# rail-berkeley/serl

Measured on AMD Instinct MI355X. Metric: learner grad-steps/sec (DrQ, bs256, 2x128x128 img), higher is better.
Workload: dtype f32 (trunk convs as split-fp16 MFMA x3, fp32 accumulate; <=1e-6 vs fp64); 1 GPU; async_drq_sim (DrQ, ResNet-10 frozen trunk, REDQ-10 critic); workload_key=drq, global_batch=256, per_gpu_batch=256, cameras=2, state_dim=24, act_dim=6, replay_capacity=200000, replay_fill=20000, parallelism=dp1, encoder=resnet-pretrained, trunk_passes_per_grad_step=2, trunk_arithmetic=f16x3, schedule=trunk(i+1) overlapped with update(i) on a 2nd stream; gather(i+2) on a 3rd

## Files before the change

serl_amd/csrc/heads.hip:

```cpp
#include <algorithm>
#include <cstdlib>

#include "heads.h"
#include "jaxrng.h"
#include "ln_stats.h"
#include "prof.h"

namespace serl {

long g_chain_launches = 0;
#define SERL_LAUNCH_CHAIN(...) do { ++g_chain_launches; hipLaunchKernelGGL(__VA_ARGS__); } while (0)

typedef float f32x16 __attribute__((ext_vector_type(16)));

constexpr int kGBM = 64, kGBN = 64, kGBK = 32, kGP = 36, kGPT = 68;
constexpr int kGTile = kGBM * kGP;
static_assert(kGBK * kGPT <= kGTile, "the [k][row] layout must fit the tile");
typedef float f32x4 __attribute__((ext_vector_type(4)));
typedef float f32x4u __attribute__((ext_vector_type(4), aligned(4)));

__device__ __forceinline__ f32x4 ld4(const float* p, int valid) {
  f32x4 v = {0.f, 0.f, 0.f, 0.f};
  if (valid >= 4) {
    v = *reinterpret_cast<const f32x4u*>(p);
// ... 1072 lines not shown
  for (int i = 0; i < n; ++i) {
    mv.v[i] = vs[i];
    gx = std::max(gx, cdiv(vs[i].D, 64));
    gy = std::max(gy, vs[i].groups);
  }
  SERL_LAUNCH_CHAIN(colsum3_kernel, dim3(gx, gy, n), dim3(512), 0, stream, mv);
  SERL_HIP(hipGetLastError());
  return SERL_OK;
}

int colsum3(const float* dg, const float* xhat, const float* dpre, int groups, int rows_per_group, int D,
            float* o_gamma, float* o_beta, float* o_bias, long gstride, hipStream_t stream) {
  const Colsum3Args v{dg, xhat, dpre, groups, rows_per_group, D, o_gamma, o_beta, o_bias, gstride, 0};
  return colsum3_multi(&v, 1, stream);
}

__global__ __launch_bounds__(256) void sle_fwd_kernel(Multi<SleFwdArgs> mv, float keep_scale, int N, int HW, int Cc,
                                                     long xs, long ks, long ms, long fs) {
  const long e = (long)blockIdx.x * 256 + threadIdx.x;
  if (e >= (long)N * Cc) return;
  const SleFwdArgs& v = mv.v[blockIdx.z];
  const float* x = v.x + blockIdx.y * xs;
  const float* K = v.K + blockIdx.y * ks;
  float* f = v.f + blockIdx.y * fs;
  const uint8_t* mask = v.mask ? v.mask + blockIdx.y * ms : nullptr;
  const int n = (int)(e / Cc), c = (int)(e - (long)n * Cc);
  float acc[8] = {0, 0, 0, 0, 0, 0, 0, 0};
#pragma unroll 4
  for (int hw = 0; hw < HW; ++hw) {
    const float xv = x[((long)n * HW + hw) * Cc + c];
    const float4 k0 = *reinterpret_cast<const float4*>(K + ((long)hw * Cc + c) * 8);
    const float4 k1 = *reinterpret_cast<const float4*>(K + ((long)hw * Cc + c) * 8 + 4);
    acc[0] += xv * k0.x; acc[1] += xv * k0.y; acc[2] += xv * k0.z; acc[3] += xv * k0.w;
    acc[4] += xv * k1.x; acc[5] += xv * k1.y; acc[6] += xv * k1.z; acc[7] += xv * k1.w;
  }
  float* o = f + (long)n * Cc * 8 + (long)c * 8;
  if (mask) {
    const uint8_t* m = mask + (long)n * Cc * 8 + (long)c * 8;
#pragma unroll
    for (int j = 0; j < 8; ++j) acc[j] = m[j] ? acc[j] * keep_scale : 0.f;
  }
  *reinterpret_cast<float4*>(o) = make_float4(acc[0], acc[1], acc[2], acc[3]);
  *reinterpret_cast<float4*>(o + 4) = make_float4(acc[4], acc[5], acc[6], acc[7]);
}

int sle_fwd_multi(const SleFwdArgs* vs, int n, float keep_scale, int N, int HW, int Cc, int groups, long x_gs, long k_gs,
                  long mask_gs, long f_gs, hipStream_t stream) {
  SERL_REQUIRE(n >= 1 && n <= kMaxMulti, "bad instance count %d", n);
  Multi<SleFwdArgs> mv{};
  for (int i = 0; i < n; ++i) mv.v[i] = vs[i];
  SERL_LAUNCH_CHAIN(sle_fwd_kernel, dim3(cdiv((long)N * Cc, 256), groups, n), dim3(256), 0, stream, mv, keep_scale, N,
                     HW, Cc, x_gs, k_gs, mask_gs, f_gs);
  SERL_HIP(hipGetLastError());
  return SERL_OK;
}


__device__ __forceinline__ void proprio_row(const ProprioArgs& a, int S, int row, int lane) {
  float v = a.b[lane];
  for (int s0 = 0; s0 < S; s0 += 64) {
    const float mine = (s0 + lane < S) ? a.state[(long)row * S + s0 + lane] : 0.f;
    const int cnt = min(64, S - s0);
    int s = 0;
    for (; s + 8 <= cnt; s += 8) {
      float w[8];
#pragma unroll
      for (int j = 0; j < 8; ++j) w[j] = a.W[(s0 + s + j) * 64 + lane];
#pragma unroll
      for (int j = 0; j < 8; ++j) v += __shfl(mine, s + j) * w[j];
    }
    for (; s < cnt; ++s) v += __shfl(mine, s) * a.W[(s0 + s) * 64 + lane];
  }
  float s1 = v, s2 = v * v;
  wave_sum2(s1, s2);
  float mean, rstd;
  ln_mean_rstd<64>(s1, s2, mean, rstd);
  const float xh = (v - mean) * rstd;
  a.y[(long)row * a.ld_y + lane] = tanhf(xh * a.gamma[lane] + a.beta[lane]);
  if (a.xhat) a.xhat[(long)row * 64 + lane] = xh;
  if (a.rstd && lane == 0) a.rstd[row] = rstd;
  if (a.copy_dst && lane < a.copy_cols) a.copy_dst[(long)row * a.ld_copy_dst + lane] = a.copy_src[(long)row * a.ld_copy_src + lane];
}

template <int kSleNb>
__global__ __launch_bounds__(256) void sle_proprio_fwd_kernel(Multi<SleFwdArgs> mv, Multi<ProprioArgs> pv, int has_proprio,
                                                              float keep_scale, unsigned keep_thr, float keep_p, int N, int HW, int Cc,
                                                              long xs, long ks, long ms, long fs, int S, int nb_sle) {
  if ((int)blockIdx.x >= nb_sle) {
    if (!has_proprio || blockIdx.y != 0) return;
    const int row = ((int)blockIdx.x - nb_sle) * 4 + (threadIdx.x >> 6);
    if (row < N) proprio_row(pv.v[blockIdx.z], S, row, threadIdx.x & 63);
    return;
  }
  const SleFwdArgs& v = mv.v[blockIdx.z];
  const int cblocks = (Cc + 255) / 256;
  const int c = ((int)blockIdx.x % cblocks) * 256 + threadIdx.x, n0 = ((int)blockIdx.x / cblocks) * kSleNb;
  if (c >= Cc) return;
  const float* x = v.x + blockIdx.y * xs + (long)n0 * HW * Cc + c;
  const float* K = v.K + blockIdx.y * ks + (long)c * 8;
  const int ns = min(kSleNb, N - n0);
  float acc[kSleNb][8];
#pragma unroll
  for (int s = 0; s < kSleNb; ++s)
#pragma unroll
    for (int j = 0; j < 8; ++j) acc[s][j] = 0.f;
  for (int hw0 = 0; hw0 < HW; hw0 += 4) {
    float4 k0[4], k1[4];
#pragma unroll
    for (int i = 0; i < 4; ++i) {
      const int hw = min(hw0 + i, HW - 1);
      k0[i] = *reinterpret_cast<const float4*>(K + (long)hw * Cc * 8);
      k1[i] = *reinterpret_cast<const float4*>(K + (long)hw * Cc * 8 + 4);
    }
    float xv[kSleNb][4];
#pragma unroll
    for (int s = 0; s < kSleNb; ++s)
#pragma unroll
      for (int i = 0; i < 4; ++i) xv[s][i] = x[((long)min(s, ns - 1) * HW + min(hw0 + i, HW - 1)) * Cc];
#pragma unroll
    for (int i = 0; i < 4; ++i) {
      if (hw0 + i < HW) {
#pragma unroll
        for (int s = 0; s < kSleNb; ++s) {
          acc[s][0] += xv[s][i] * k0[i].x; acc[s][1] += xv[s][i] * k0[i].y; acc[s][2] += xv[s][i] * k0[i].z; acc[s][3] += xv[s][i] * k0[i].w;
          acc[s][4] += xv[s][i] * k1[i].x; acc[s][5] += xv[s][i] * k1[i].y; acc[s][6] += xv[s][i] * k1[i].z; acc[s][7] += xv[s][i] * k1[i].w;
        }
      }
    }
  }
  float* f = v.f + blockIdx.y * fs + (long)n0 * Cc * 8 + (long)c * 8;
  const uint8_t* mask = v.mask ? v.mask + blockIdx.y * ms + (long)n0 * Cc * 8 + (long)c * 8 : nullptr;
#pragma unroll
  for (int s = 0; s < kSleNb; ++s) {
    if (s >= ns) break;
    if (mask) {
      const uint8_t* m = mask + (long)s * Cc * 8;
#pragma unroll
      for (int j = 0; j < 8; ++j) acc[s][j] = m[j] ? acc[s][j] * keep_scale : 0.f;
    } else if (v.gen == 2) {
      const uint32_t k0 = v.tf_key[blockIdx.y][0], k1 = v.tf_key[blockIdx.y][1];
      const uint64_t rowlen = (uint64_t)Cc * 8ull, total = (uint64_t)v.tf_rows * rowlen;
      const uint64_t e0 = (uint64_t)(v.tf_row0 + n0 + s) * rowlen + (uint64_t)c * 8ull;
#pragma unroll
      for (int j = 0; j < 8; ++j)
        acc[s][j] = bits_to_unit(random_bits_at(k0, k1, total, e0 + (uint64_t)j)) < keep_p ? acc[s][j] * keep_scale : 0.f;
    } else if (v.gen) {
      const uint64_t ctr = (((uint64_t)blockIdx.y * (uint64_t)v.rows_global + (uint64_t)(v.row_offset + n0 + s)) * (uint64_t)Cc + (uint64_t)c) * 3ull;
      const uint64_t h0 = mix64(v.seed ^ mix64(ctr)), h1 = mix64(v.seed ^ mix64(ctr + 1)), h2 = mix64(v.seed ^ mix64(ctr + 2));
      const unsigned u[8] = {(unsigned)(h0 & 0xFFFFFF), (unsigned)((h0 >> 24) & 0xFFFFFF), (unsigned)((h0 >> 48) | ((h1 & 0xFF) << 16)),
                             (unsigned)((h1 >> 8) & 0xFFFFFF), (unsigned)((h1 >> 32) & 0xFFFFFF), (unsigned)((h1 >> 56) | ((h2 & 0xFFFF) << 8)),
                             (unsigned)((h2 >> 16) & 0xFFFFFF), (unsigned)(h2 >> 40)};
#pragma unroll
      for (int j = 0; j < 8; ++j) acc[s][j] = u[j] < keep_thr ? acc[s][j] * keep_scale : 0.f;
    }
    *reinterpret_cast<float4*>(f + (long)s * Cc * 8) = make_float4(acc[s][0], acc[s][1], acc[s][2], acc[s][3]);
    *reinterpret_cast<float4*>(f + (long)s * Cc * 8 + 4) = make_float4(acc[s][4], acc[s][5], acc[s][6], acc[s][7]);
  }
}

int sle_proprio_fwd_multi(const SleFwdArgs* vs, const ProprioArgs* ps, int n, float keep, int N, int HW, int Cc, int groups, long x_gs,
                          long k_gs, long mask_gs, long f_gs, int state_dim, hipStream_t stream) {
  SERL_REQUIRE(n >= 1 && n <= kMaxMulti, "bad instance count %d", n);
  Multi<SleFwdArgs> mv{};
  Multi<ProprioArgs> pv{};
  for (int i = 0; i < n; ++i) {
    mv.v[i] = vs[i];
    if (ps) { pv.v[i] = ps[i]; SERL_REQUIRE(!ps[i].copy_dst || ps[i].copy_cols <= 64, "copy_cols > 64"); }
  }
  const int nb = N <= 64 ? 2 : 8;
  const int nb_sle = cdiv(Cc, 256) * cdiv(N, nb), nb_prop = ps ? cdiv(N, 4) : 0;
  if (nb == 2)
    SERL_LAUNCH_CHAIN(sle_proprio_fwd_kernel<2>, dim3(nb_sle + nb_prop, groups, n), dim3(256), 0, stream, mv, pv, ps ? 1 : 0,
                      1.0f / keep, (unsigned)(keep * 16777216.0f), keep, N, HW, Cc, x_gs, k_gs, mask_gs, f_gs, state_dim, nb_sle);
  else
    SERL_LAUNCH_CHAIN(sle_proprio_fwd_kernel<8>, dim3(nb_sle + nb_prop, groups, n), dim3(256), 0, stream, mv, pv, ps ? 1 : 0,
                      1.0f / keep, (unsigned)(keep * 16777216.0f), keep, N, HW, Cc, x_gs, k_gs, mask_gs, f_gs, state_dim, nb_sle);
  SERL_HIP(hipGetLastError());
  return SERL_OK;
}

__global__ __launch_bounds__(256) void sle_bwd_kernel(const float* x, const float* df, float* partial, int N,
                                                     int HW, int Cc, int nsplit, long x_gs, long df_gs, long part_gs) {
  const int c = blockIdx.x * 256 + threadIdx.x, hw = blockIdx.y, sp = blockIdx.z % nsplit, grp = blockIdx.z / nsplit;
  if (c >= Cc) return;
  x += grp * x_gs; df += grp * df_gs; partial += grp * part_gs;
  const int per = (N + nsplit - 1) / nsplit;
  const int nb = sp * per, ne = min(N, nb + per);
  float acc[8] = {0, 0, 0, 0, 0, 0, 0, 0};
  for (int n = nb; n < ne; ++n) {
    const float xv = x[((long)n * HW + hw) * Cc + c];
    const float4 d0 = *reinterpret_cast<const float4*>(df + (long)n * Cc * 8 + (long)c * 8);
    const float4 d1 = *reinterpret_cast<const float4*>(df + (long)n * Cc * 8 + (long)c * 8 + 4);
    acc[0] += xv * d0.x; acc[1] += xv * d0.y; acc[2] += xv * d0.z; acc[3] += xv * d0.w;
    acc[4] += xv * d1.x; acc[5] += xv * d1.y; acc[6] += xv * d1.z; acc[7] += xv * d1.w;
  }
  float* o = partial + (((long)sp * HW + hw) * Cc + c) * 8;
  *reinterpret_cast<float4*>(o) = make_float4(acc[0], acc[1], acc[2], acc[3]);
  *reinterpret_cast<float4*>(o + 4) = make_float4(acc[4], acc[5], acc[6], acc[7]);
}

__global__ __launch_bounds__(256) void sle_bwd_fused_kernel(const float* x, const float* df, float* partial, int N, int HW, int Cc,
                                                           int nsplit, long x_gs, long df_gs, long part_gs, float* out, long out_gs,
                                                           int* ctr) {
  __shared__ int s_last;
  const int c = blockIdx.x * 256 + threadIdx.x, hw = blockIdx.y, sp = blockIdx.z % nsplit, grp = blockIdx.z / nsplit;
  x += grp * x_gs; df += grp * df_gs; partial += grp * part_gs;
  const int per = (N + nsplit - 1) / nsplit;
  const int nb = sp * per, ne = min(N, nb + per);
  float acc[8] = {0, 0, 0, 0, 0, 0, 0, 0};
  if (c < Cc) {
    for (int n = nb; n < ne; ++n) {
      const float xv = x[((long)n * HW + hw) * Cc + c];
      const float4 d0 = *reinterpret_cast<const float4*>(df + (long)n * Cc * 8 + (long)c * 8);
      const float4 d1 = *reinterpret_cast<const float4*>(df + (long)n * Cc * 8 + (long)c * 8 + 4);
      acc[0] += xv * d0.x; acc[1] += xv * d0.y; acc[2] += xv * d0.z; acc[3] += xv * d0.w;
      acc[4] += xv * d1.x; acc[5] += xv * d1.y; acc[6] += xv * d1.z; acc[7] += xv * d1.w;
    }
    const __amdgpu_buffer_rsrc_t rs = rsrc_of(partial);
    const long o = (((long)sp * HW + hw) * Cc + c) * 8;
    __builtin_amdgcn_raw_buffer_store_b128(__builtin_bit_cast(u32x4_t, (f32x4){acc[0], acc[1], acc[2], acc[3]}), rs, (int)(o * 4), 0, kSc1);
    __builtin_amdgcn_raw_buffer_store_b128(__builtin_bit_cast(u32x4_t, (f32x4){acc[4], acc[5], acc[6], acc[7]}), rs, (int)(o * 4 + 16), 0, kSc1);
  }
  if (!arrive_is_last(ctr + ((long)grp * HW + hw) * gridDim.x + blockIdx.x, nsplit, &s_last)) return;
  if (c >= Cc) return;
  const __amdgpu_buffer_rsrc_t rs = rsrc_of(partial);
  f32x4 s0 = {0.f, 0.f, 0.f, 0.f}, s1 = {0.f, 0.f, 0.f, 0.f};
  for (int s = 0; s < nsplit; ++s) {
    const long o = (((long)s * HW + hw) * Cc + c) * 8;
    s0 += ld_sc1(rs, o);
    s1 += ld_sc1(rs, o + 4);
  }
  float* o = out + grp * out_gs + ((long)hw * Cc + c) * 8;
  *reinterpret_cast<f32x4*>(o) = s0;
  *reinterpret_cast<f32x4*>(o + 4) = s1;
}

int sle_bwd_fused(const float* x, const float* df, float* partial, int N, int HW, int Cc, int nsplit, int groups,
                  long x_gs, long df_gs, long part_gs, float* out, long out_gs, int* ctr, hipStream_t stream) {
  SERL_REQUIRE((long)nsplit * HW * Cc * 8 * 4 < (1L << 31), "SLE partial sums exceed 2 GB");
  SERL_LAUNCH_CHAIN(sle_bwd_fused_kernel, dim3(cdiv(Cc, 256), HW, nsplit * groups), dim3(256), 0, stream, x, df, partial, N,
                     HW, Cc, nsplit, x_gs, df_gs, part_gs, out, out_gs, ctr);
  SERL_HIP(hipGetLastError());
  return SERL_OK;
}

int sle_bwd(const float* x, const float* df, float* partial, int N, int HW, int Cc, int nsplit, int groups,
            long x_gs, long df_gs, long part_gs, hipStream_t stream) {
  SERL_LAUNCH_CHAIN(sle_bwd_kernel, dim3(cdiv(Cc, 256), HW, nsplit * groups), dim3(256), 0, stream, x, df, partial, N,
                     HW, Cc, nsplit, x_gs, df_gs, part_gs);
  SERL_HIP(hipGetLastError());
  return SERL_OK;
}

__global__ __launch_bounds__(256) void critic_loss_kernel(LossArgs L) {
  __shared__ float red[4][256];
  critic_loss_body(L, red);
}

// ... 374 lines not shown
```

serl_amd/csrc/trunk_f16x3.hip:

```cpp
#include "trunk_f16x3_elementwise.h"

namespace serl {

static int resident_workgroups(hipStream_t stream) {
  thread_local hipStream_t last = nullptr;
  thread_local int last_n = -1;
  if (last_n >= 0 && last == stream) return last_n;
  int dev = 0, n = 0;
  hipDeviceProp_t prop;
  if (hipGetDevice(&dev) == hipSuccess && hipGetDeviceProperties(&prop, dev) == hipSuccess) n = prop.multiProcessorCount;
  uint32_t mask[16] = {0};
  if (hipExtStreamGetCUMask(stream, 16, mask) == hipSuccess) {
    int m = 0;
    for (uint32_t w : mask) m += __builtin_popcount(w);
    if (m > 0 && (n == 0 || m < n)) n = m;
  } else {
    (void)hipGetLastError();
  }
  last = stream; last_n = n;
  return n;
}

static_assert(kStageFilters[0] % 64 == 0 && kStageFilters[1] % 64 == 0 && kStageFilters[2] % 64 == 0 && kStageFilters[3] % 64 == 0,
              "conv channels unsupported (Cin % 32, Cout % 64)");
// ... 31 lines not shown
    const int tiles_n = a.Cout / 64;
    if (fuse && a.P == 256) {
      l.fused = 2;
    } else if (fuse && a.P % 256 == 0 && fused_can_wait(resident, a.P / 256 * tiles_n)) {
      l.fused = 1; l.expected = a.P / 256; l.group = a.P / 256 * tiles_n;
    }
    l.stagger = (l.fused && a.M / 256 * tiles_n >= 1024) ? 5 : 0;
  } else if (dma_ok) {
    l.kern = 'D'; l.cfg = cfg;
    const int tn = cfg == 0 ? 2 : 1, tiles_n = a.Cout / (64 * tn);
    if (pmode == 1 && cfg == 4) pmode = 3;
    if (fuse && pmode == 0 && a.P % 128 == 0 && a.Cout / kGnGroups <= 64 * tn && fused_can_wait(resident, a.P / 128 * tiles_n)) {
      l.fused = 1; l.expected = a.P / 128; l.group = a.P / 128 * tiles_n;
    } else if (fuse && pmode == 0 && a.P == 64 && a.M % 128 == 0 && tn == 2 && a.Cout / kGnGroups == 64) {
      l.fused = 2;
    } else if (fuse && pmode == 2 && a.P == 16 && a.M % 128 == 0 && tn == 2 && a.Cout / kGnGroups == 128) {
      l.fused = 2;
    }
    l.proj = proj && pmode != 3 && a.KH == 3 && a.stride == 2 && a.pad == 0 && a.padw == 0;
  } else {
    l.kern = 'R'; l.cfg = cfg;
  }
  l.pmode = pmode;
  l.pad = a.pad; l.padw = a.padw;
  return l;
}

static int plan_pass(TrunkPlan& p, const TrunkDims& d, int N, const TrunkPacked& pk, const bool (&has_proj)[kTrunkStages], int resident,
                     bool fuse, bool proj_fuse) {
  p = TrunkPlan{};
  p.images = N; p.fuse = fuse;
  const bool fuse_pool = d.h[0] % 16 == 0 && d.w[0] % 16 == 0;
  const bool complete_pool = fuse_pool && N >= 512 && N % 512 == 0;
  p.pool = complete_pool ? 2 : (fuse_pool ? 1 : 0);
  const ConvArgs b0 = conv_geom(d, N, 0, 0);
  p.raw_b0 = complete_pool && fuse && !has_proj[0] && rowslab_shape_ok(b0) && b0.Cin <= 128 && pk.blk[0][0].dma && pk.blk[0][1].dma &&
             b0.P % 256 == 0 && fused_can_wait(resident, b0.P / 256 * (b0.Cout / 64));
  for (int i = 0; i < kTrunkStages; ++i) {
    TrunkPlan::L* l = p.conv[i];
    const bool raw = i == 0 && p.raw_b0;
    l[0] = plan_conv(conv_geom(d, N, i, 0), pk.blk[i][0].dma, pk.zero, fuse, resident, raw, has_proj[i] && proj_fuse && pk.blk[i][2].dma);
    if (l[0].proj) {
      l[2] = l[0];
      l[2].kern = 'F'; l[2].fused = 0;
    } else if (has_proj[i]) {
      l[2] = plan_conv(conv_geom(d, N, i, 2), pk.blk[i][2].dma, pk.zero, false, resident, false, false);
    }
    l[1] = plan_conv(conv_geom(d, N, i, 1), pk.blk[i][1].dma, pk.zero, fuse, resident, false, false);
    SERL_REQUIRE(!raw || (l[0].kern == 'S' && l[0].fused && l[1].fused),
                 "block 0 was planned on the fused row-slab path");
  }
  return SERL_OK;
}

template <int WM, int WN, int TM, int TN, int DEEP>
static void launch_igemm(ConvArgsB ab, int pmode, hipStream_t stream) {
  constexpr int BM = 32 * TM * WM, BN = 32 * TN * WN;
  ab.c.tiles_m = cdiv(ab.c.M, BM); ab.c.tiles_n = ab.c.Cout / BN;
  const dim3 grid(ab.c.tiles_m * ab.c.tiles_n), block(256);
  const size_t lds = (size_t)2 * (2 * BM * 64 + 2 * BN * 64);
  if (pmode == 0) hipLaunchKernelGGL((conv_igemm_f16x3_kernel<WM, WN, TM, TN, 0, DEEP>), grid, block, lds, stream, ab);
  else if (pmode == 1) hipLaunchKernelGGL((conv_igemm_f16x3_kernel<WM, WN, TM, TN, 1, DEEP>), grid, block, lds, stream, ab);
  else if (pmode == 2) hipLaunchKernelGGL((conv_igemm_f16x3_kernel<WM, WN, TM, TN, 2, DEEP>), grid, block, lds, stream, ab);
  else hipLaunchKernelGGL((conv_igemm_f16x3_kernel<WM, WN, TM, TN, 3, DEEP>), grid, block, lds, stream, ab);
}
template <int TN, bool PROJ>
static void launch_dma(ConvArgsB ab, int pmode, const uint8_t* zero_page, const ConvProjB& pj, hipStream_t stream) {
  ab.c.tiles_m = cdiv(ab.c.M, 128); ab.c.tiles_n = ab.c.Cout / (64 * TN);
  const dim3 grid(ab.c.tiles_m * ab.c.tiles_n), block(256);
  const size_t lds = (size_t)4 * (128 * 64 + 64 * TN * 64);
  if (pmode == 0) hipLaunchKernelGGL((conv_dma_f16x3_kernel<TN, 0, PROJ>), grid, block, lds, stream, ab, zero_page, pj);
  else if (pmode == 1) hipLaunchKernelGGL((conv_dma_f16x3_kernel<TN, 1, PROJ>), grid, block, lds, stream, ab, zero_page, pj);
  else if (pmode == 2 || PROJ) hipLaunchKernelGGL((conv_dma_f16x3_kernel<TN, 2, PROJ>), grid, block, lds, stream, ab, zero_page, pj);
  else if constexpr (!PROJ) hipLaunchKernelGGL((conv_dma_f16x3_kernel<TN, 3, false>), grid, block, lds, stream, ab, zero_page, pj);
}
static int launch_conv_f16x3(const char* tag, const TrunkPlan::L& l, const ConvArgs& a, PackedConvWeights w, const FuseArgs& fz,
                             const ConvProjB& pj, const uint8_t* zero_page, hipStream_t stream) {
  ConvArgsB ab{};
  ab.c = a;
  ab.whi = w.hi; ab.wlo = w.lo; ab.winv = w.inv; ab.wdma = w.dma; ab.K = a.KH * a.KW * a.Cin;
  ab.wprio = trunk_wave_prio(a.N);
  ab.stagger = l.stagger;
  if (l.fused) { ab.fz = fz; ab.fz.expected = l.expected; ab.fz.group = l.group; }
  {
    ProfScope prof(tag, stream);
    if (l.kern == 'S') {
      ab.c.tiles_m = a.M / 256; ab.c.tiles_n = a.Cout / 64;
      const dim3 grid(ab.c.tiles_m * ab.c.tiles_n), block(256);
      if (l.raw)
        hipLaunchKernelGGL(conv3x3_rowslab_f16x3_kernel, grid, block, (size_t)kRowslabLds, stream, ab);
      else if (l.fused) hipLaunchKernelGGL(conv3x3_slabdma_f16x3_kernel<true>, grid, block, (size_t)kSlabDmaLds, stream, ab, zero_page);
      else hipLaunchKernelGGL(conv3x3_slabdma_f16x3_kernel<false>, grid, block, (size_t)kSlabDmaLds, stream, ab, zero_page);
    } else if (l.kern == 'D') {
      if (l.proj) {
        if (l.cfg == 0) launch_dma<2, true>(ab, l.pmode, zero_page, pj, stream);
        else launch_dma<1, true>(ab, l.pmode, zero_page, pj, stream);
      } else if (l.cfg == 0) launch_dma<2, false>(ab, l.pmode, zero_page, ConvProjB{}, stream);
      else launch_dma<1, false>(ab, l.pmode, zero_page, ConvProjB{}, stream);
    } else {
      if (l.cfg == 0) launch_igemm<2, 2, 2, 2, 0>(ab, l.pmode, stream);
      else if (l.cfg == 1) launch_igemm<4, 1, 2, 2, 0>(ab, l.pmode, stream);
      else if (l.cfg == 4) launch_igemm<2, 2, 2, 1, 3>(ab, l.pmode, stream);
      else launch_igemm<2, 2, 1, 1, 3>(ab, l.pmode, stream);
    }
  }
  SERL_HIP(hipGetLastError());
  if (l.pmode == 3) {
    hipLaunchKernelGGL(gn_stats_kernel_b, dim3(a.N * kGnGroups), dim3(256), 0, stream, a.out, a.stats, a.P, a.Cout);
    SERL_HIP(hipGetLastError());
  }
  return SERL_OK;
}

__global__ __launch_bounds__(256) void zero_sys_kernel(void* p, long n16) {
  const __amdgpu_buffer_rsrc_t r = __builtin_amdgcn_make_buffer_rsrc(p, 0, 0x7fffffff, 0x00020000);
  const u32x4 z = {0u, 0u, 0u, 0u};
  for (long i = (long)blockIdx.x * 256 + threadIdx.x; i < n16; i += (long)gridDim.x * 256)
    __builtin_amdgcn_raw_buffer_store_b128(z, r, (int)(i * 16), 0, 17 );
}

static std::mutex g_fused_mu;
static hipStream_t g_fused_stream = nullptr;
static hipEvent_t g_fused_done = nullptr;
static bool g_fused_any = false, g_fused_open = false;
static bool claim_fused_pass(hipStream_t stream) {
  std::lock_guard<std::mutex> lk(g_fused_mu);
  if (g_fused_any && g_fused_stream != stream &&
      (g_fused_open || (g_fused_done && hipEventQuery(g_fused_done) == hipErrorNotReady))) return false;
  (void)hipGetLastError();
  g_fused_stream = stream;
  g_fused_any = g_fused_open = true;
  return true;
}
static void fused_pass_issued(hipStream_t stream) {
  std::lock_guard<std::mutex> lk(g_fused_mu);
  if (g_fused_stream != stream) return;
  g_fused_open = false;
  if (!g_fused_done && hipEventCreateWithFlags(&g_fused_done, hipEventDisableTiming) != hipSuccess) { g_fused_done = nullptr; return; }
  (void)hipEventRecord(g_fused_done, stream);
}

int trunk_forward_f16x3(const TrunkWeights& w, TrunkWorkspace& ws, TrunkPacked& pk, const uint8_t* frames, int N,
                        float* feats_out, hipStream_t stream, int stage_begin, int stage_end) {
  const TrunkDims& d = ws.d;
  const TrunkPlan& plan = ws.plan;
  auto stats_of = [&](int layer) { return ws.stats + (size_t)layer * ws.max_images * kGnGroups * 2; };
  int rc;
  if (stage_begin < 0) {
    const char* gf = getenv("SERL_GN_FUSE");
    const char* pf = getenv("SERL_PROJ_FUSE");
    const bool fuse = !(gf && gf[0] == '0') && claim_fused_pass(stream);
    const bool has_proj[kTrunkStages] = {w.blk[0].proj != nullptr, w.blk[1].proj != nullptr, w.blk[2].proj != nullptr,
                                         w.blk[3].proj != nullptr};
    const int resident = fuse ? resident_workgroups(stream) : 0;
    if ((rc = plan_pass(ws.plan, d, N, pk, has_proj, resident, fuse, !(pf && pf[0] == '0')))) return rc;
    auto zero_sys = [&](void* p, size_t bytes) -> int {
      for (size_t off = 0; off < bytes; off += (size_t)1 << 30) {
        const long n16 = (long)(std::min(bytes - off, (size_t)1 << 30) / 16);
        hipLaunchKernelGGL(zero_sys_kernel, dim3((unsigned)std::min<long>(cdiv(n16, 256), 512)), dim3(256), 0, stream,
                           (void*)((uint8_t*)p + off), n16);
        SERL_HIP(hipGetLastError());
      }
      return SERL_OK;
    };
    if ((rc = zero_sys(ws.stats, ws.stats_sync_bytes))) return rc;
    const GnxEpoch ep = gnx_next_epoch(ws.epoch);
// ... 107 lines not shown
```

serl_amd/csrc/trunk_f16x3_dma.h:

```cpp
#pragma once
#include "trunk_f16x3_igemm.h"

namespace serl {

template <int TN, int PMODE>
__device__ __forceinline__ void dma_tile_epilogue(const ConvArgsB& ab, f32x16 (&acc)[2][TN], f32x16 (&accx)[2][TN], int m0, int n0,
                                                  int bn, int wm, int wn, int li, int lh) {
  constexpr int TM = 2, WROWS = 64, WCOLS = 32 * TN;
  const ConvArgs& a = ab.c;
  const int wrow0 = m0 + wm * WROWS;
  if (ab.wprio == 2) __builtin_amdgcn_s_setprio(1);
  float winv[TN];
#pragma unroll
  for (int tn = 0; tn < TN; ++tn) winv[tn] = ab.winv[n0 + wn * WCOLS + tn * 32 + li];
#pragma unroll
  for (int tm = 0; tm < TM; ++tm)
#pragma unroll
    for (int tn = 0; tn < TN; ++tn)
#pragma unroll
      for (int r = 0; r < 16; ++r) acc[tm][tn][r] = (acc[tm][tn][r] + accx[tm][tn][r] * kLoInv) * winv[tn];
  FusedResidual<TM, TN> fres;
  if ((PMODE == 0 || PMODE == 2) && ab.fz.mode) fused_load_residual<TM, TN>(ab, fres, wrow0, n0 + wn * WCOLS, li, lh);
  if (!ab.fz.mode) {
#pragma unroll
// ... 92 lines not shown
#pragma unroll
        for (int r = 8 * (sl & 1); r < 8 * (sl & 1) + 8; ++r) { const float v = acc[sl >> 1][tn][r]; ps += v; pq += v * v; }
      s4[sl] = (double)ps; q4[sl] = (double)pq;
#pragma unroll
      for (int off = 1; off < 64; off <<= 1) { s4[sl] += __shfl_xor(s4[sl], off); q4[sl] += __shfl_xor(q4[sl], off); }
    }
    const int wave = wm * 2 + wn;
    if (li == 0 && lh == 0) {
#pragma unroll
      for (int sl = 0; sl < 4; ++sl) { s_x[wave][sl][0] = s4[sl]; s_x[wave][sl][1] = q4[sl]; }
    }
    __syncthreads();
    float lmean[4], lrstd[4];
#pragma unroll
    for (int sl = 0; sl < 4; ++sl) {
      const double ss = s_x[wm * 2][sl][0] + s_x[wm * 2 + 1][sl][0], qq = s_x[wm * 2][sl][1] + s_x[wm * 2 + 1][sl][1];
      const double mean = ss * ab.fz.gn.inv_count, m2 = qq * ab.fz.gn.inv_count;
      const float var = fmaxf((float)(m2 - mean * mean), 0.f);
      lmean[sl] = (float)mean; lrstd[sl] = rsqrtf(var + 1e-5f);
    }
    fused_gn_store<TM, TN, 4>(ab, acc, fres, wrow0 / a.P, wrow0, n0 + wn * WCOLS, li, lh, lmean, lrstd);
  }
}

template <int TN, int PMODE>
__device__ __forceinline__ void dma_proj_epilogue(const ConvArgsB& ab, const ConvProjB& pj, f32x16 (&acc)[2][TN], f32x16 (&accx)[2][TN],
                                                  int m0, int n0, int wm, int wn, int li, int lh) {
  static_assert(PMODE != 3, "the fused projection takes its statistics in the kernel");
  constexpr int TM = 2, WROWS = 64, WCOLS = 32 * TN;
  const ConvArgs& a = ab.c;
  const int wrow0 = m0 + wm * WROWS;
  float winv[TN];
#pragma unroll
  for (int tn = 0; tn < TN; ++tn) winv[tn] = pj.winv[n0 + wn * WCOLS + tn * 32 + li];
#pragma unroll
  for (int tm = 0; tm < TM; ++tm)
#pragma unroll
    for (int tn = 0; tn < TN; ++tn)
#pragma unroll
      for (int r = 0; r < 16; ++r) acc[tm][tn][r] = (acc[tm][tn][r] + accx[tm][tn][r] * kLoInv) * winv[tn];
#pragma unroll
  for (int tm = 0; tm < TM; ++tm)
#pragma unroll
    for (int r = 0; r < 16; ++r) {
      const int m = wrow0 + tm * 32 + (r & 3) + 8 * (r >> 2) + 4 * lh;
      if (m < a.M) {
        float* o = pj.out + (size_t)m * a.Cout + n0 + wn * WCOLS + li;
#pragma unroll
        for (int tn = 0; tn < TN; ++tn) o[32 * tn] = acc[tm][tn][r];
      }
    }
  const int gsize = a.Cout / kGnGroups;
  constexpr int ROWS = PMODE == 0 ? WROWS : (PMODE == 1 ? 32 : 16);
  constexpr int NSLOT = WROWS / ROWS;
#pragma unroll
  for (int slot = 0; slot < NSLOT; ++slot) {
    const int mrow = wrow0 + slot * ROWS;
    const bool valid = mrow < a.M;
    const int n = valid ? mrow / a.P : 0;
    double* stp = pj.stats + (size_t)n * kGnGroups * 2;
#pragma unroll
    for (int tn = 0; tn < TN; ++tn) {
      float s = 0.f, q = 0.f;
#pragma unroll
      for (int tm = 0; tm < TM; ++tm)
#pragma unroll
        for (int r = 0; r < 16; ++r) {
          const int row = tm * 32 + 8 * (r >> 2);
          if (row / ROWS == slot) {
            const float v = acc[tm][tn][r];
            s += v;
            q += v * v;
          }
        }
      stats_flush(s, q, stp, n0 + wn * WCOLS + tn * 32 + li, gsize, valid, false);
    }
  }
}

typedef __attribute__((address_space(3))) void lds_void_t;
typedef __attribute__((address_space(1))) const void gbl_void_t;

template <int TN, int PMODE, bool PROJ = false>
__global__ __launch_bounds__(256, 2) void conv_dma_f16x3_kernel(ConvArgsB ab, const uint8_t* zero_page, ConvProjB pj) {
  static_assert(!PROJ || PMODE != 3, "the fused projection takes its statistics in the kernel");
  constexpr int NS = 4;
  const ConvArgs& a = ab.c;
  constexpr int TM = 2, WROWS = 64, WCOLS = 32 * TN, BM = 128, BN = 2 * WCOLS;
  constexpr int A_BYTES = BM * 64, SLOT = A_BYTES + BN * 64;
  constexpr int A_PIECES = BM / 16 / 4;
  constexpr int B_PIECES = BN / 16 / 4;
  constexpr int PIECES = A_PIECES + B_PIECES;
  extern __shared__ __attribute__((aligned(16))) uint8_t smemb[];
  const int tid = threadIdx.x, lane = tid & 63, wave = __builtin_amdgcn_readfirstlane(tid >> 6);
  const int wm = wave >> 1, wn = wave & 1;
  if (ab.wprio) __builtin_amdgcn_s_setprio(3);
  const int id = (ab.fz.mode && ab.fz.expected) ? fused_tile(ab.fz, gridDim.x) : xcd_remap((int)blockIdx.x, gridDim.x);
  const int bn = id % a.tiles_n, bm = id / a.tiles_n;
  const int m0 = bm * BM, n0 = bn * BN;
  const int ntaps = a.KH * a.KW;
  unsigned rbase[A_PIECES], rmask[A_PIECES];
  const uint8_t* in_bytes = reinterpret_cast<const uint8_t*>(a.in);
#pragma unroll
  for (int q = 0; q < A_PIECES; ++q) {
    const int row = (q * 4 + wave) * 16 + (lane >> 2);
    const int u = (lane & 3) ^ ((row >> 2) & 3);
    const int m = m0 + row;
    rbase[q] = 0; rmask[q] = 0;
    if (m < a.M) {
      const int n = m / a.P, rem = m - n * a.P;
      const int oy = rem / a.Wo, ox = rem - oy * a.Wo;
      rbase[q] = (unsigned)((((long)(n * a.Hi + oy * a.stride) * a.Wi + ox * a.stride) * a.Cin) * 4 + u * 16);
      for (int t = 0; t < ntaps; ++t) {
        const int iy = oy * a.stride - a.pad + t / a.KW, ix = ox * a.stride - a.padw + t % a.KW;
        if ((unsigned)iy < (unsigned)a.Hi && (unsigned)ix < (unsigned)a.Wi) rmask[q] |= 1u << t;
      }
    }
  }
  const int nslots = ntaps * (a.Cin >> 4);
  constexpr bool with_proj = PROJ;
  int run_nslots = with_proj ? (a.Cin >> 4) : nslots, run_kw = with_proj ? 1 : a.KW;
  const uint8_t* wsrc[B_PIECES];
#pragma unroll
  for (int q = 0; q < B_PIECES; ++q) {
    const int prow = (q * 4 + wave) * 16 + (lane >> 2);
    wsrc[q] = reinterpret_cast<const uint8_t*>(with_proj ? pj.wdma : ab.wdma) + (size_t)((n0 + prow) >> 6) * run_nslots * 4096 +
              ((prow & 63) << 6) + ((lane & 3) << 4);
  }
  int l_tap = 0, l_ky = 0, l_kx = 0, l_ci0 = 0, l_slot = 0;
  const uint8_t* zp = zero_page + (lane & 3) * 16;
  int nx_tap = 0, nx_toff = 0, nx_k = 0, nx_ring = 0;
#define SERL_RING_PIECE(PI)                                                                                    \
  {                                                                                                            \
    uint8_t* st_ = smemb + nx_ring * SLOT;                                                                     \
    if ((PI) < A_PIECES) {                                                                                     \
      const int q = (PI) < A_PIECES ? (PI) : 0;                                                                \
      const bool ok = (rmask[q] >> nx_tap) & 1u;                                                               \
      const uint8_t* src = ok ? in_bytes + (size_t)rbase[q] + (long)nx_toff : zp;                              \
      __builtin_amdgcn_global_load_lds((gbl_void_t*)src, (lds_void_t*)(st_ + (q * 4 + wave) * 1024), 16, 0, 0); \
    } else {                                                                                                   \
      const int q = (PI) >= A_PIECES ? (PI) - A_PIECES : 0;                                                    \
      __builtin_amdgcn_global_load_lds((gbl_void_t*)(wsrc[q] + (size_t)nx_k * 4096),                           \
                                       (lds_void_t*)(st_ + A_BYTES + (q * 4 + wave) * 1024), 16, 0, 0);        \
    }                                                                                                          \
  }
#define SERL_RING_NEXT(RING)                                                                                   \
  {                                                                                                            \
    nx_tap = l_tap; nx_k = l_slot; nx_ring = (RING);                                                           \
    nx_toff = (((l_ky - a.pad) * a.Wi + (l_kx - a.padw)) * a.Cin + l_ci0) * 4;                                 \
    if (l_slot + 1 < run_nslots) {                                                                             \
      ++l_slot;                                                                                                \
      l_ci0 += 16;                                                                                             \
      if (l_ci0 == a.Cin) { l_ci0 = 0; ++l_tap; if (++l_kx == run_kw) { l_kx = 0; ++l_ky; } }                  \
    }                                                                                                          \
  }
  f32x16 acc[TM][TN], accx[TM][TN];
#pragma unroll
  for (int tm = 0; tm < TM; ++tm)
#pragma unroll
    for (int tn = 0; tn < TN; ++tn)
#pragma unroll
      for (int r = 0; r < 16; ++r) { acc[tm][tn][r] = 0.f; accx[tm][tn][r] = 0.f; }
  const int li = lane & 31, lh = lane >> 5;
  int ahi_off[TM], alo_off[TM], bhi_off[TN], blo_off[TN];
#pragma unroll
  for (int tm = 0; tm < TM; ++tm) {
    const int row = wm * WROWS + tm * 32 + li, sw = (row >> 2) & 3;
    ahi_off[tm] = row * 64 + (((2 * lh) ^ sw) << 4);
    alo_off[tm] = row * 64 + (((2 * lh + 1) ^ sw) << 4);
  }
#pragma unroll
  for (int tn = 0; tn < TN; ++tn) {
    const int row = wn * WCOLS + tn * 32 + li, sw = (row >> 2) & 3;
    bhi_off[tn] = A_BYTES + row * 64 + ((lh ^ sw) << 4);
    blo_off[tn] = A_BYTES + row * 64 + (((2 + lh) ^ sw) << 4);
  }
  constexpr int GROUPS = TM * TN;
  f16x8 fa[2][2 * TM], fb[2][2 * TN];
#define SERL_RING_READ(SET, ST)                                                                \
  {                                                                                            \
    _Pragma("unroll") for (int tm = 0; tm < TM; ++tm) {                                        \
      fa[SET][2 * tm] = *reinterpret_cast<const f16x8*>((ST) + ahi_off[tm]);                   \
      fa[SET][2 * tm + 1] = *reinterpret_cast<const f16x8*>((ST) + alo_off[tm]);               \
    }                                                                                          \
    _Pragma("unroll") for (int tn = 0; tn < TN; ++tn) {                                        \
      fb[SET][2 * tn] = *reinterpret_cast<const f16x8*>((ST) + bhi_off[tn]);                   \
      fb[SET][2 * tn + 1] = *reinterpret_cast<const f16x8*>((ST) + blo_off[tn]);               \
    }                                                                                          \
  }
#define SERL_RING_READ1(SET, ST, I)                                                            \
  {                                                                                            \
    if ((I) < 2 * TM) {                                                                        \
      const int tm_ = (I) >> 1;                                                                \
      fa[SET][I] = *reinterpret_cast<const f16x8*>((ST) + (((I) & 1) ? alo_off[tm_ < TM ? tm_ : 0] : ahi_off[tm_ < TM ? tm_ : 0])); \
    } else {                                                                                   \
      const int j_ = (I) - 2 * TM, tn_ = j_ >> 1;                                              \
      fb[SET][j_ < 2 * TN ? j_ : 0] = *reinterpret_cast<const f16x8*>((ST) + ((j_ & 1) ? blo_off[tn_ < TN ? tn_ : 0] : bhi_off[tn_ < TN ? tn_ : 0])); \
    }                                                                                          \
  }
#define SERL_RING_ITER(C, CUR)                                                                 \
  {                                                                                            \
    __builtin_amdgcn_sched_barrier(0);                                                         \
    asm volatile("s_waitcnt vmcnt(%0) lgkmcnt(0)" ::"n"((NS - 2) * PIECES) : "memory");        \
    asm volatile("s_barrier" ::: "memory");                                                    \
    __builtin_amdgcn_sched_barrier(0);                                                         \
    SERL_RING_NEXT((C) % NS);                                                                  \
    const uint8_t* stn = smemb + (((C) + 1) % NS) * SLOT;                                      \
    constexpr int NREAD = 2 * TM + 2 * TN, RPG = (NREAD + GROUPS - 1) / GROUPS;                \
    _Pragma("unroll") for (int tm = 0; tm < TM; ++tm)                                          \
      _Pragma("unroll") for (int tn = 0; tn < TN; ++tn) {                                      \
        const int g = tm * TN + tn;                                                            \
        __builtin_amdgcn_sched_barrier(0);                                                     \
        accx[tm][tn] = __builtin_amdgcn_mfma_f32_32x32x16_f16(fa[CUR][2 * tm + 1], fb[CUR][2 * tn], accx[tm][tn], 0, 0, 0); \
        _Pragma("unroll") for (int i = 0; i < RPG; ++i) if (g * RPG + i < NREAD) SERL_RING_READ1(1 - (CUR), stn, g * RPG + i) \
        __builtin_amdgcn_sched_barrier(0);                                                     \
        acc[tm][tn] = __builtin_amdgcn_mfma_f32_32x32x16_f16(fa[CUR][2 * tm], fb[CUR][2 * tn], acc[tm][tn], 0, 0, 0); \
        _Pragma("unroll") for (int pi = 0; pi < PIECES; ++pi)                                  \
          if (pi % GROUPS == g) SERL_RING_PIECE(pi)                         \
        __builtin_amdgcn_sched_barrier(0);                                                     \
        accx[tm][tn] = __builtin_amdgcn_mfma_f32_32x32x16_f16(fa[CUR][2 * tm], fb[CUR][2 * tn + 1], accx[tm][tn], 0, 0, 0); \
      }                                                                                        \
  }
#define SERL_RING_RUN()                                                                        \
  {                                                                                            \
    l_tap = 0; l_ky = 0; l_kx = 0; l_ci0 = 0; l_slot = 0;                                      \
    _Pragma("unroll") for (int p = 0; p < NS; ++p) {                                           \
      SERL_RING_NEXT(p);                                                                       \
      _Pragma("unroll") for (int pi = 0; pi < PIECES; ++pi) SERL_RING_PIECE(pi)                \
    }                                                                                          \
    asm volatile("s_waitcnt vmcnt(%0)" ::"n"((NS - 1) * PIECES) : "memory");                   \
    asm volatile("s_barrier" ::: "memory");                                                    \
    SERL_RING_READ(0, smemb);                                                                  \
    for (int c = 0; c < run_nslots; c += 2) {      \
      SERL_RING_ITER(c, 0);                                                                    \
      SERL_RING_ITER(c + 1, 1);                                                                \
    }                                                                                          \
    asm volatile("s_waitcnt vmcnt(0)" ::: "memory");                                           \
  }
  if constexpr (PROJ) {
    {
      SERL_RING_RUN();
      dma_proj_epilogue<TN, PMODE>(ab, pj, acc, accx, m0, n0, wm, wn, li, lh);
#pragma unroll
      for (int tm = 0; tm < TM; ++tm)
#pragma unroll
        for (int tn = 0; tn < TN; ++tn)
#pragma unroll
          for (int r = 0; r < 16; ++r) { acc[tm][tn][r] = 0.f; accx[tm][tn][r] = 0.f; }
      asm volatile("s_waitcnt vmcnt(0) lgkmcnt(0)" ::: "memory");
      asm volatile("s_barrier" ::: "memory");
      run_nslots = nslots; run_kw = a.KW;
#pragma unroll
      for (int q = 0; q < B_PIECES; ++q) {
        const int prow = (q * 4 + wave) * 16 + (lane >> 2);
        wsrc[q] = reinterpret_cast<const uint8_t*>(ab.wdma) + (size_t)((n0 + prow) >> 6) * nslots * 4096 + ((prow & 63) << 6) + ((lane & 3) << 4);
      }
    }
  }
  SERL_RING_RUN();
#undef SERL_RING_RUN
#undef SERL_RING_ITER
#undef SERL_RING_READ
#undef SERL_RING_READ1
#undef SERL_RING_PIECE
#undef SERL_RING_NEXT
  dma_tile_epilogue<TN, PMODE>(ab, acc, accx, m0, n0, bn, wm, wn, li, lh);
}

}
```

Baseline: 434.7 grad-steps/s.

## Cut VGPR pressure in DMA conv kernel and retune SLE forward tiling

The DMA f16x3 conv kernel is capped at 108 VGPRs. To fit, its per-fragment and per-piece address arrays become single base offsets plus compile-time strides, and the per-lane state is rematerialized after the fused projection instead of being kept live across it. Opaque asm barriers stop the compiler from hoisting that recomputation back. Separately, the SLE forward kernel for N>64 now uses 4 samples by 2 pixels per block instead of 8 by 4, which lowers register use and gives more blocks. A host-side check rejects residual mode on projection-fused convs, and the kernel now assumes that mode cannot occur.

```diff
diff --git a/serl_amd/csrc/heads.hip b/serl_amd/csrc/heads.hip
--- a/serl_amd/csrc/heads.hip
+++ b/serl_amd/csrc/heads.hip
@@ -1178,7 +1178,7 @@
   if (a.copy_dst && lane < a.copy_cols) a.copy_dst[(long)row * a.ld_copy_dst + lane] = a.copy_src[(long)row * a.ld_copy_src + lane];
 }
 
-template <int kSleNb>
+template <int kSleNb, int kPx>
 __global__ __launch_bounds__(256) void sle_proprio_fwd_kernel(Multi<SleFwdArgs> mv, Multi<ProprioArgs> pv, int has_proprio,
                                                               float keep_scale, unsigned keep_thr, float keep_p, int N, int HW, int Cc,
                                                               long xs, long ks, long ms, long fs, int S, int nb_sle) {
@@ -1200,21 +1200,21 @@
   for (int s = 0; s < kSleNb; ++s)
 #pragma unroll
     for (int j = 0; j < 8; ++j) acc[s][j] = 0.f;
-  for (int hw0 = 0; hw0 < HW; hw0 += 4) {
-    float4 k0[4], k1[4];
-#pragma unroll
-    for (int i = 0; i < 4; ++i) {
+  for (int hw0 = 0; hw0 < HW; hw0 += kPx) {
+    float4 k0[kPx], k1[kPx];
+#pragma unroll
+    for (int i = 0; i < kPx; ++i) {
       const int hw = min(hw0 + i, HW - 1);
       k0[i] = *reinterpret_cast<const float4*>(K + (long)hw * Cc * 8);
       k1[i] = *reinterpret_cast<const float4*>(K + (long)hw * Cc * 8 + 4);
     }
-    float xv[kSleNb][4];
+    float xv[kSleNb][kPx];
 #pragma unroll
     for (int s = 0; s < kSleNb; ++s)
 #pragma unroll
-      for (int i = 0; i < 4; ++i) xv[s][i] = x[((long)min(s, ns - 1) * HW + min(hw0 + i, HW - 1)) * Cc];
-#pragma unroll
-    for (int i = 0; i < 4; ++i) {
+      for (int i = 0; i < kPx; ++i) xv[s][i] = x[((long)min(s, ns - 1) * HW + min(hw0 + i, HW - 1)) * Cc];
+#pragma unroll
+    for (int i = 0; i < kPx; ++i) {
       if (hw0 + i < HW) {
 #pragma unroll
         for (int s = 0; s < kSleNb; ++s) {
@@ -1263,13 +1263,13 @@
     mv.v[i] = vs[i];
     if (ps) { pv.v[i] = ps[i]; SERL_REQUIRE(!ps[i].copy_dst || ps[i].copy_cols <= 64, "copy_cols > 64"); }
   }
-  const int nb = N <= 64 ? 2 : 8;
+  const int nb = N <= 64 ? 2 : 4;
   const int nb_sle = cdiv(Cc, 256) * cdiv(N, nb), nb_prop = ps ? cdiv(N, 4) : 0;
   if (nb == 2)
-    SERL_LAUNCH_CHAIN(sle_proprio_fwd_kernel<2>, dim3(nb_sle + nb_prop, groups, n), dim3(256), 0, stream, mv, pv, ps ? 1 : 0,
+    SERL_LAUNCH_CHAIN((sle_proprio_fwd_kernel<2, 4>), dim3(nb_sle + nb_prop, groups, n), dim3(256), 0, stream, mv, pv, ps ? 1 : 0,
                       1.0f / keep, (unsigned)(keep * 16777216.0f), keep, N, HW, Cc, x_gs, k_gs, mask_gs, f_gs, state_dim, nb_sle);
   else
-    SERL_LAUNCH_CHAIN(sle_proprio_fwd_kernel<8>, dim3(nb_sle + nb_prop, groups, n), dim3(256), 0, stream, mv, pv, ps ? 1 : 0,
+    SERL_LAUNCH_CHAIN((sle_proprio_fwd_kernel<4, 2>), dim3(nb_sle + nb_prop, groups, n), dim3(256), 0, stream, mv, pv, ps ? 1 : 0,
                       1.0f / keep, (unsigned)(keep * 16777216.0f), keep, N, HW, Cc, x_gs, k_gs, mask_gs, f_gs, state_dim, nb_sle);
   SERL_HIP(hipGetLastError());
   return SERL_OK;
diff --git a/serl_amd/csrc/trunk_f16x3.hip b/serl_amd/csrc/trunk_f16x3.hip
--- a/serl_amd/csrc/trunk_f16x3.hip
+++ b/serl_amd/csrc/trunk_f16x3.hip
@@ -137,6 +137,7 @@
   ab.wprio = trunk_wave_prio(a.N);
   ab.stagger = l.stagger;
   if (l.fused) { ab.fz = fz; ab.fz.expected = l.expected; ab.fz.group = l.group; }
+  SERL_REQUIRE(!l.proj || ab.fz.mode < 2, "%s: a conv with a fused projection cannot take a residual (mode %d)", tag, (int)ab.fz.mode);
   {
     ProfScope prof(tag, stream);
     if (l.kern == 'S') {
diff --git a/serl_amd/csrc/trunk_f16x3_dma.h b/serl_amd/csrc/trunk_f16x3_dma.h
--- a/serl_amd/csrc/trunk_f16x3_dma.h
+++ b/serl_amd/csrc/trunk_f16x3_dma.h
@@ -198,8 +198,9 @@
 typedef __attribute__((address_space(1))) const void gbl_void_t;
 
 template <int TN, int PMODE, bool PROJ = false>
-__global__ __launch_bounds__(256, 2) void conv_dma_f16x3_kernel(ConvArgsB ab, const uint8_t* zero_page, ConvProjB pj) {
+__global__ __launch_bounds__(256, 2) __attribute__((amdgpu_num_vgpr(108))) void conv_dma_f16x3_kernel(ConvArgsB ab, const uint8_t* zero_page, ConvProjB pj) {
   static_assert(!PROJ || PMODE != 3, "the fused projection takes its statistics in the kernel");
+  if constexpr (PROJ) __builtin_assume(ab.fz.mode < 2);
   constexpr int NS = 4;
   const ConvArgs& a = ab.c;
   constexpr int TM = 2, WROWS = 64, WCOLS = 32 * TN, BM = 128, BN = 2 * WCOLS;
@@ -217,32 +218,30 @@
   const int ntaps = a.KH * a.KW;
   unsigned rbase[A_PIECES], rmask[A_PIECES];
   const uint8_t* in_bytes = reinterpret_cast<const uint8_t*>(a.in);
-#pragma unroll
-  for (int q = 0; q < A_PIECES; ++q) {
-    const int row = (q * 4 + wave) * 16 + (lane >> 2);
-    const int u = (lane & 3) ^ ((row >> 2) & 3);
-    const int m = m0 + row;
-    rbase[q] = 0; rmask[q] = 0;
-    if (m < a.M) {
-      const int n = m / a.P, rem = m - n * a.P;
-      const int oy = rem / a.Wo, ox = rem - oy * a.Wo;
-      rbase[q] = (unsigned)((((long)(n * a.Hi + oy * a.stride) * a.Wi + ox * a.stride) * a.Cin) * 4 + u * 16);
-      for (int t = 0; t < ntaps; ++t) {
-        const int iy = oy * a.stride - a.pad + t / a.KW, ix = ox * a.stride - a.padw + t % a.KW;
-        if ((unsigned)iy < (unsigned)a.Hi && (unsigned)ix < (unsigned)a.Wi) rmask[q] |= 1u << t;
-      }
-    }
-  }
+  auto piece_state = [&](int ln) {
+#pragma unroll
+    for (int q = 0; q < A_PIECES; ++q) {
+      const int row = (q * 4 + wave) * 16 + (ln >> 2);
+      const int u = (ln & 3) ^ ((row >> 2) & 3);
+      const int m = m0 + row;
+      rbase[q] = 0; rmask[q] = 0;
+      if (m < a.M) {
+        const int n = m / a.P, rem = m - n * a.P;
+        const int oy = rem / a.Wo, ox = rem - oy * a.Wo;
+        rbase[q] = (unsigned)((((long)(n * a.Hi + oy * a.stride) * a.Wi + ox * a.stride) * a.Cin) * 4 + u * 16);
+        for (int t = 0; t < ntaps; ++t) {
+          const int iy = oy * a.stride - a.pad + t / a.KW, ix = ox * a.stride - a.padw + t % a.KW;
+          if ((unsigned)iy < (unsigned)a.Hi && (unsigned)ix < (unsigned)a.Wi) rmask[q] |= 1u << t;
+        }
+      }
+    }
+  };
+  piece_state(lane);
   const int nslots = ntaps * (a.Cin >> 4);
   constexpr bool with_proj = PROJ;
   int run_nslots = with_proj ? (a.Cin >> 4) : nslots, run_kw = with_proj ? 1 : a.KW;
-  const uint8_t* wsrc[B_PIECES];
-#pragma unroll
-  for (int q = 0; q < B_PIECES; ++q) {
-    const int prow = (q * 4 + wave) * 16 + (lane >> 2);
-    wsrc[q] = reinterpret_cast<const uint8_t*>(with_proj ? pj.wdma : ab.wdma) + (size_t)((n0 + prow) >> 6) * run_nslots * 4096 +
-              ((prow & 63) << 6) + ((lane & 3) << 4);
-  }
+  const uint8_t* wbase = reinterpret_cast<const uint8_t*>(with_proj ? pj.wdma : ab.wdma) + (size_t)(n0 >> 6) * run_nslots * 4096;
+  const unsigned wlane = ((wave * 16 + (lane >> 2)) << 6) + ((lane & 3) << 4);
   int l_tap = 0, l_ky = 0, l_kx = 0, l_ci0 = 0, l_slot = 0;
   const uint8_t* zp = zero_page + (lane & 3) * 16;
   int nx_tap = 0, nx_toff = 0, nx_k = 0, nx_ring = 0;
@@ -256,7 +255,7 @@
       __builtin_amdgcn_global_load_lds((gbl_void_t*)src, (lds_void_t*)(st_ + (q * 4 + wave) * 1024), 16, 0, 0); \
     } else {                                                                                                   \
       const int q = (PI) >= A_PIECES ? (PI) - A_PIECES : 0;                                                    \
-      __builtin_amdgcn_global_load_lds((gbl_void_t*)(wsrc[q] + (size_t)nx_k * 4096),                           \
+      __builtin_amdgcn_global_load_lds((gbl_void_t*)(wbase + ((size_t)q * run_nslots + nx_k) * 4096 + wlane),   \
                                        (lds_void_t*)(st_ + A_BYTES + (q * 4 + wave) * 1024), 16, 0, 0);        \
     }                                                                                                          \
   }
@@ -277,41 +276,39 @@
     for (int tn = 0; tn < TN; ++tn)
 #pragma unroll
       for (int r = 0; r < 16; ++r) { acc[tm][tn][r] = 0.f; accx[tm][tn][r] = 0.f; }
-  const int li = lane & 31, lh = lane >> 5;
-  int ahi_off[TM], alo_off[TM], bhi_off[TN], blo_off[TN];
-#pragma unroll
-  for (int tm = 0; tm < TM; ++tm) {
-    const int row = wm * WROWS + tm * 32 + li, sw = (row >> 2) & 3;
-    ahi_off[tm] = row * 64 + (((2 * lh) ^ sw) << 4);
-    alo_off[tm] = row * 64 + (((2 * lh + 1) ^ sw) << 4);
-  }
-#pragma unroll
-  for (int tn = 0; tn < TN; ++tn) {
-    const int row = wn * WCOLS + tn * 32 + li, sw = (row >> 2) & 3;
-    bhi_off[tn] = A_BYTES + row * 64 + ((lh ^ sw) << 4);
-    blo_off[tn] = A_BYTES + row * 64 + (((2 + lh) ^ sw) << 4);
-  }
+  int li = lane & 31, lh = lane >> 5;
+  int ahi_off, alo_off, bhi_off, blo_off;
+  auto frag_state = [&](int ln) {
+    const int li_ = ln & 31, lh_ = ln >> 5;
+    const int arow = wm * WROWS + li_, asw = (arow >> 2) & 3;
+    ahi_off = arow * 64 + (((2 * lh_) ^ asw) << 4);
+    alo_off = arow * 64 + (((2 * lh_ + 1) ^ asw) << 4);
+    const int brow = wn * WCOLS + li_, bsw = (brow >> 2) & 3;
+    bhi_off = A_BYTES + brow * 64 + ((lh_ ^ bsw) << 4);
+    blo_off = A_BYTES + brow * 64 + (((2 + lh_) ^ bsw) << 4);
+  };
+  frag_state(lane);
   constexpr int GROUPS = TM * TN;
   f16x8 fa[2][2 * TM], fb[2][2 * TN];
 #define SERL_RING_READ(SET, ST)                                                                \
   {                                                                                            \
     _Pragma("unroll") for (int tm = 0; tm < TM; ++tm) {                                        \
-      fa[SET][2 * tm] = *reinterpret_cast<const f16x8*>((ST) + ahi_off[tm]);                   \
-      fa[SET][2 * tm + 1] = *reinterpret_cast<const f16x8*>((ST) + alo_off[tm]);               \
+      fa[SET][2 * tm] = *reinterpret_cast<const f16x8*>((ST) + ahi_off + tm * 2048);                   \
+      fa[SET][2 * tm + 1] = *reinterpret_cast<const f16x8*>((ST) + alo_off + tm * 2048);               \
     }                                                                                          \
     _Pragma("unroll") for (int tn = 0; tn < TN; ++tn) {                                        \
-      fb[SET][2 * tn] = *reinterpret_cast<const f16x8*>((ST) + bhi_off[tn]);                   \
-      fb[SET][2 * tn + 1] = *reinterpret_cast<const f16x8*>((ST) + blo_off[tn]);               \
+      fb[SET][2 * tn] = *reinterpret_cast<const f16x8*>((ST) + bhi_off + tn * 2048);                   \
+      fb[SET][2 * tn + 1] = *reinterpret_cast<const f16x8*>((ST) + blo_off + tn * 2048);               \
     }                                                                                          \
   }
 #define SERL_RING_READ1(SET, ST, I)                                                            \
   {                                                                                            \
     if ((I) < 2 * TM) {                                                                        \
       const int tm_ = (I) >> 1;                                                                \
-      fa[SET][I] = *reinterpret_cast<const f16x8*>((ST) + (((I) & 1) ? alo_off[tm_ < TM ? tm_ : 0] : ahi_off[tm_ < TM ? tm_ : 0])); \
+      fa[SET][I] = *reinterpret_cast<const f16x8*>((ST) + (((I) & 1) ? alo_off : ahi_off) + tm_ * 2048); \
     } else {                                                                                   \
       const int j_ = (I) - 2 * TM, tn_ = j_ >> 1;                                              \
-      fb[SET][j_ < 2 * TN ? j_ : 0] = *reinterpret_cast<const f16x8*>((ST) + ((j_ & 1) ? blo_off[tn_ < TN ? tn_ : 0] : bhi_off[tn_ < TN ? tn_ : 0])); \
+      fb[SET][j_ < 2 * TN ? j_ : 0] = *reinterpret_cast<const f16x8*>((ST) + ((j_ & 1) ? blo_off : bhi_off) + tn_ * 2048); \
     }                                                                                          \
   }
 #define SERL_RING_ITER(C, CUR)                                                                 \
@@ -356,7 +353,11 @@
   if constexpr (PROJ) {
     {
       SERL_RING_RUN();
-      dma_proj_epilogue<TN, PMODE>(ab, pj, acc, accx, m0, n0, wm, wn, li, lh);
+      {
+        int li_p = li, lh_p = lh;
+        asm volatile("" : "+v"(li_p), "+v"(lh_p));
+        dma_proj_epilogue<TN, PMODE>(ab, pj, acc, accx, m0, n0, wm, wn, li_p, lh_p);
+      }
 #pragma unroll
       for (int tm = 0; tm < TM; ++tm)
 #pragma unroll
@@ -366,14 +367,20 @@
       asm volatile("s_waitcnt vmcnt(0) lgkmcnt(0)" ::: "memory");
       asm volatile("s_barrier" ::: "memory");
       run_nslots = nslots; run_kw = a.KW;
-#pragma unroll
-      for (int q = 0; q < B_PIECES; ++q) {
-        const int prow = (q * 4 + wave) * 16 + (lane >> 2);
-        wsrc[q] = reinterpret_cast<const uint8_t*>(ab.wdma) + (size_t)((n0 + prow) >> 6) * nslots * 4096 + ((prow & 63) << 6) + ((lane & 3) << 4);
-      }
+      int ln = lane;
+      asm volatile("" : "+v"(ln));
+      piece_state(ln);
+      frag_state(ln);
+      zp = zero_page + (ln & 3) * 16;
+      wbase = reinterpret_cast<const uint8_t*>(ab.wdma) + (size_t)(n0 >> 6) * nslots * 4096;
     }
   }
   SERL_RING_RUN();
+  if constexpr (PROJ) {
+    int le = lane;
+    asm volatile("" : "+v"(le));
+    li = le & 31; lh = le >> 5;
+  }
 #undef SERL_RING_RUN
 #undef SERL_RING_ITER
 #undef SERL_RING_READ
```

Measured after the change: 442.2 grad-steps/s, median of 6. 1.7% higher.
